# 0xPolygonZero/proof-protocol-decoder

Measured on NVIDIA B200. Metric: mpt_nodes_keccak_hashed_per_sec, higher is better.
Workload: dtype u64

## Files before the change

proof_protocol_decoder_b200/csrc/txn_core.h:

```cpp
#pragma once
#include <cstdint>

#include "../../include/ppd_flat.h"
#include "arena.h"

#if defined(__CUDACC__)
#define PPD_HD __host__ __device__ __forceinline__
#define PPD_INLINE
#else
#define PPD_HD
#define PPD_INLINE inline
#endif

namespace ppd {
namespace txn {

static const uint32_t T_UNCHANGED = 0xfffffffeu;
static const uint32_t ST_ABSENT = 0xfffffffeu;
static const uint32_t NONE = 0xfffffffdu;
static const uint32_t HASH_BASE = 0x80000000u, HASH_END = 0xf0000000u;
static const uint32_t MARK_SLOTS_T = 16;
static const uint32_t PATH_CAP = 15;
static const uint32_t OWNER_TXN_TRIE = 0xffffff01u, OWNER_RECEIPT_TRIE = 0xffffff02u, OWNER_STATE_TRIE = 0xffffff03u;
static const uint32_t TRF_STATE_WRITE = 0x100u;
// ... 202 lines not shown
#define PPD_PREFETCH(p) asm volatile("prefetch.global.L1 [%0];" ::"l"(p))
#define PPD_FENCE_BLOCK() __threadfence_block()
#define PPD_ATOMIC_SUB(p, x) atomicSub((p), (x))
#define PPD_ATOMIC_ADD(p, x) atomicAdd((p), (x))
#define PPD_ATOMIC_MAX(p, x) atomicMax((p), (x))
#define PPD_ATOMIC_CAS(p, c, x) atomicCAS((p), (c), (x))
#else
PPD_HD PPD_INLINE uint32_t host_atomic_add(uint32_t* p, uint32_t x) {
  uint32_t o = *p;
  *p = o + x;
  return o;
}
PPD_HD PPD_INLINE uint32_t host_atomic_max(uint32_t* p, uint32_t x) {
  uint32_t o = *p;
  if (x > o) *p = x;
  return o;
}
PPD_HD PPD_INLINE uint32_t host_atomic_cas(uint32_t* p, uint32_t c, uint32_t x) {
  uint32_t o = *p;
  if (o == c) *p = x;
  return o;
}
#define PPD_FENCE_BLOCK() ((void)0)
#define PPD_PREFETCH(p) ((void)0)
#define PPD_ATOMIC_SUB(p, x) ppd::txn::host_atomic_add((p), 0u - (x))
#define PPD_ATOMIC_ADD(p, x) ppd::txn::host_atomic_add((p), (x))
#define PPD_ATOMIC_MAX(p, x) ppd::txn::host_atomic_max((p), (x))
#define PPD_ATOMIC_CAS(p, c, x) ppd::txn::host_atomic_cas((p), (c), (x))
#endif

PPD_HD PPD_INLINE void raise(const View& v, uint32_t why, uint32_t txn) {
  if (PPD_ATOMIC_CAS(&v.cur->flag, 0u, why) == 0u) v.cur->flag_txn = txn;
}

PPD_HD PPD_INLINE uint32_t key_nib(const View& v, uint32_t koff, uint32_t i) {
  const uint32_t b = v.key_pool[koff + (i >> 1)];
  return (i & 1) ? (b & 15u) : (b >> 4);
}
PPD_HD PPD_INLINE uint32_t lvl(const View& v, uint32_t n) { return (n == NODE_EMPTY || n >= HASH_BASE) ? 0u : (uint32_t)v.level[n]; }
PPD_HD PPD_INLINE uint32_t kind_of(const View& v, uint32_t n) { return is_hash_id(n) ? (uint32_t)NK_HASH : (v.nodes[n].w0 & 0xffu); }
PPD_HD PPD_INLINE uint32_t w0(uint32_t kind, uint32_t start, uint32_t len) { return kind | (start << 8) | (len << 16); }

PPD_HD PPD_INLINE uint32_t push_node(const View& v, const NodeRec& r, uint32_t lv) {
  uint32_t id = PPD_ATOMIC_ADD(SCR(v).a_nodes, 1u);
  if (id >= v.cap_nodes) {
    raise(v, TXF_NODES_FULL, 0);
    id = v.cap_nodes - 1;
// ... 72 lines not shown
PPD_HD PPD_INLINE uint32_t child_at(const View& v, const NodeRec& br, uint32_t nib) {
  const uint32_t mask = br.a1 & 0xffffu, bit = 1u << nib;
  if (!(mask & bit)) return NODE_EMPTY;
#if defined(__CUDA_ARCH__)
  return v.child_pool[br.a0 + __popc(mask & (bit - 1))];
#else
  return v.child_pool[br.a0 + __builtin_popcount(mask & (bit - 1))];
#endif
}
PPD_HD PPD_INLINE uint32_t popc16(uint32_t m) {
#if defined(__CUDA_ARCH__)
  return __popc(m & 0xffffu);
#else
  return (uint32_t)__builtin_popcount(m & 0xffffu);
#endif
}

struct NL {
  uint32_t id, lv;
};
PPD_HD PPD_INLINE NL new_leaf_for(const View& v, const SOp& o, uint32_t start) {
  const uint32_t len = o.klen - start;
  if (o.kind == OP_PUT_ACCOUNT) {
    const uint32_t src = v.accounts[o.a1].storage_src;
    const uint32_t lv = src == NODE_EMPTY ? 0u : lvl(v, src) + 1u;
    return NL{push_node(v, NodeRec{w0(NK_LEAF_ACCOUNT, start, len), o.koff, o.a1, 0}, lv), lv};
  }
  return NL{push_node(v, NodeRec{w0(NK_LEAF, start, len), o.koff, o.a1, o.a2}, 0), 0};
}
PPD_HD PPD_INLINE NL new_ext(const View& v, uint32_t koff, uint32_t start, uint32_t len, NL child) {
  return NL{push_node(v, NodeRec{w0(NK_EXT, start, len), koff, child.id, 0}, child.lv + 1u), child.lv + 1u};
}
PPD_HD PPD_INLINE uint32_t new_root(const View& v, uint32_t child) {
  return push_node(v, NodeRec{w0(NK_ROOT, 0, 0), 0, child, 0}, child == NODE_EMPTY ? 0u : lvl(v, child) + 1u);
}
PPD_HD PPD_INLINE NL releaf(const View& v, uint32_t leaf, uint32_t leaf_lv, uint32_t koff, uint32_t start, uint32_t len) {
  NodeRec r = v.nodes[leaf];
  r.w0 = w0(r.w0 & 0xffu, start, len);
  r.a0 = koff;
  return NL{push_node(v, r, leaf_lv), leaf_lv};
}
PPD_HD PPD_INLINE NL new_branch16(const View& v, const uint32_t* kids, uint32_t lv) {
  uint32_t mask = 0, k = 0;
  for (uint32_t i = 0; i < 16; i++)
    if (kids[i] != NODE_EMPTY) mask |= 1u << i, k++;
  const uint32_t base = alloc_children(v, k);
  for (uint32_t i = 0, j = 0; i < 16; i++)
    if (kids[i] != NODE_EMPTY) v.child_pool[base + j++] = kids[i];
  return NL{push_node(v, NodeRec{w0(NK_BRANCH, 0, 0), base, mask, 0}, lv), lv};
}
PPD_HD PPD_INLINE NL branch_with(const View& v, uint32_t br, uint32_t nib, NL child) {
  const NodeRec r = v.nodes[br];
  uint32_t lv = v.level[br];
  const uint32_t mask = r.a1 & 0xffffu, bit = 1u << nib;
  const uint32_t k = popc16(mask), rk = popc16(mask & (bit - 1)), has = (mask & bit) ? 1u : 0u;
  const uint32_t nk = k - has + 1u, base = alloc_children(v, nk);
  uint32_t old[16];
  for (uint32_t i = 0; i < 16; i++) old[i] = i < k ? v.child_pool[r.a0 + i] : 0u;
  for (uint32_t i = 0; i < rk; i++) v.child_pool[base + i] = old[i];
  v.child_pool[base + rk] = child.id;
  for (uint32_t i = rk + has; i < k; i++) v.child_pool[base + i - has + 1u] = old[i];
  if (child.lv + 1u > lv) lv = child.lv + 1u;
  return NL{push_node(v, NodeRec{w0(NK_BRANCH, 0, 0), base, mask | bit, 0}, lv), lv};
}
PPD_HD PPD_INLINE NL collapse_ext(const View& v, uint32_t ek, uint32_t es, uint32_t el, NL child) {
  const uint32_t k = kind_of(v, child.id);
  if (k == NK_EXT) {
    const NodeRec c = v.nodes[child.id];
    return NL{push_node(v, NodeRec{w0(NK_EXT, ((c.w0 >> 8) & 0xffu) - el, ((c.w0 >> 16) & 0xffu) + el), c.a0, c.a1, 0}, child.lv), child.lv};
  }
  if (k == NK_LEAF || k == NK_LEAF_ACCOUNT) {
    const NodeRec c = v.nodes[child.id];
    return releaf(v, child.id, child.lv, c.a0, ((c.w0 >> 8) & 0xffu) - el, ((c.w0 >> 16) & 0xffu) + el);
  }
  return new_ext(v, ek, es, el, child);
}
PPD_HD PPD_INLINE NL collapse_branch(const View& v, uint32_t koff, uint32_t pos, uint32_t nib, NL other) {
  const uint32_t k = kind_of(v, other.id);
  if (k == NK_EXT || k == NK_LEAF || k == NK_LEAF_ACCOUNT) return collapse_ext(v, 0, pos, 1, other);
  const uint32_t nb = pos / 2 + 2;
  uint32_t pk = PPD_ATOMIC_ADD(SCR(v).a_keys, nb);
  if (pk + nb > v.cap_keys) {
    raise(v, TXF_KEYS_FULL, 0);
    pk = v.cap_keys - 40;
  }
  for (uint32_t i = 0; i <= pos / 2; i++) v.key_pool[pk + i] = v.key_pool[koff + i];
  uint8_t* last = v.key_pool + pk + pos / 2;
  *last = (pos & 1) ? (uint8_t)((*last & 0xf0u) | nib) : (uint8_t)(nib << 4);
  v.key_pool[pk + pos / 2 + 1] = 0;
  return new_ext(v, pk, pos, 1, other);
}

PPD_HD PPD_INLINE NL split_at(const View& v, const SOp& o, uint32_t pos, uint32_t cp, uint32_t existing_nib, NL existing, uint32_t txn) {
  const uint32_t at = pos + cp;
  if (at >= o.klen) {
    raise(v, TXF_KEY_PREFIX, txn);
    return existing;
  }
  const uint32_t new_nib = key_nib(v, o.koff, at);
  uint32_t kids[16];
  for (int i = 0; i < 16; i++) kids[i] = NODE_EMPTY;
  const NL leaf = new_leaf_for(v, o, at + 1);
  kids[existing_nib] = existing.id;
  kids[new_nib] = leaf.id;
  const NL br = new_branch16(v, kids, (existing.lv > leaf.lv ? existing.lv : leaf.lv) + 1u);
  return cp == 0 ? br : new_ext(v, o.koff, pos, cp, br);
}
PPD_HD PPD_INLINE NL insert_one(const View& v, NL base, uint32_t depth, const SOp& o, uint32_t txn) {
  uint32_t st_node[PATH_CAP + 1];
  uint8_t st_nib[PATH_CAP + 1];
  uint32_t sp = 0, node = base.id, pos = depth;
  NL result = base;
  for (;;) {
    if (node == NODE_EMPTY) {
      result = new_leaf_for(v, o, pos);
      break;
    }
    const uint32_t k = kind_of(v, node);
    if (k == NK_HASH || k == NK_ROOT) {
      raise(v, TXF_INSERT_INTO_HASH, txn);
      return base;
    }
    const NodeRec r = v.nodes[node];
    const uint32_t ns = (r.w0 >> 8) & 0xffu, nl = (r.w0 >> 16) & 0xffu;
    if (k == NK_BRANCH) {
      if (pos >= o.klen || sp == PATH_CAP + 1) {
        raise(v, pos >= o.klen ? TXF_KEY_PREFIX : TXF_STACK, txn);
        return base;
// ... 21 lines not shown
        break;
      }
    } else {
      const uint32_t avail = o.klen - pos, m = avail < nl ? avail : nl;
      const uint32_t cp = common_prefix(v, r.a0, ns, o.koff, pos, m);
      if (cp == nl && nl == avail) {
        result = new_leaf_for(v, o, pos);
      } else if (cp == nl) {
        raise(v, TXF_KEY_PREFIX, txn);
        return base;
      } else {
        const NL existing = releaf(v, node, node == base.id ? base.lv : (uint32_t)v.level[node], r.a0, ns + cp + 1, nl - cp - 1);
        result = split_at(v, o, pos, cp, key_nib(v, r.a0, ns + cp), existing, txn);
      }
      break;
    }
  }
  while (sp) {
    sp--;
    if (st_nib[sp] == 0xff) {
      const NodeRec r = v.nodes[st_node[sp]];
      result = new_ext(v, r.a0, (r.w0 >> 8) & 0xffu, (r.w0 >> 16) & 0xffu, result);
    } else {
      result = branch_with(v, st_node[sp], st_nib[sp], result);
    }
  }
  return result;
}

struct Batch {
  const SOp* ops;
  uint32_t n;
  uint32_t base;
  uint32_t txn;
};

PPD_HD PPD_INLINE int shared_depth(const Batch& b, uint32_t i) {
  const int prev = (int)b.ops[i].lcp, next = i + 1 < b.n ? (int)b.ops[i + 1].lcp : -1;
  return prev > next ? prev : next;
}
PPD_HD PPD_INLINE uint32_t trie_root_of(const View& v, uint32_t owner) {
  if (owner == OWNER_STATE_TRIE) return v.cur->state_root;
  if (owner == OWNER_TXN_TRIE) return v.cur->txn_root;
  if (owner == OWNER_RECEIPT_TRIE) return v.cur->receipt_root;
  return v.acct[v.traces[owner].acct].storage;
}

PPD_HD PPD_INLINE PathNode& pc_at(const View& v, uint32_t idx) { return idx < SCR(v).pc_n_fast ? SCR(v).pc_fast[idx] : SCR(v).pc_slow[idx - SCR(v).pc_n_fast]; }
PPD_HD PPD_INLINE uint32_t pc_hash(uint32_t node) { return node * 2654435761u; }
PPD_HD PPD_INLINE uint32_t pc_make(const View& v, uint32_t node, const NodeRec& r, bool is_branch, uint32_t owner, uint32_t txn) {
  uint32_t idx = PPD_ATOMIC_ADD(SCR(v).pc_count, 1u);
  if (idx >= SCR(v).pc_n_fast + SCR(v).pc_n_slow) {
    raise(v, TXF_PATH_TABLE, txn);
    return NONE;
  }
  PathNode& p = pc_at(v, idx);
  p.kids[0] = r.a0, p.kids[1] = is_branch ? (r.a1 & 0xffffu) : 0x10000u;
  p.node = node, p.lv = 0, p.pending = 0, p.owner = owner, p.changed = 0;
  uint32_t h = pc_hash(node) & SCR(v).pc_map_mask;
  for (;;) {
    const uint32_t prev = PPD_ATOMIC_CAS(&SCR(v).pc_map_key[h], 0xffffffffu, node);
    if (prev == 0xffffffffu || prev == node) break;
    h = (h + 1) & SCR(v).pc_map_mask;
  }
  SCR(v).pc_map[h] = idx + 1u;
  return idx;
}
PPD_HD PPD_INLINE void pc_fill(const View& v, uint32_t idx) {
  PathNode& p = pc_at(v, idx);
  const uint32_t a0 = p.kids[0], m = p.kids[1];
  const uint32_t old_lv = v.level[p.node];
  if (m & 0x10000u) {
    p.kids[0] = T_UNCHANGED, p.kids[1] = 0;
  } else {
    const uint32_t mask = m & 0xffffu;
    uint32_t x[16];
#if defined(__CUDA_ARCH__)
#pragma unroll
#endif
    for (uint32_t nib = 0; nib < 16; nib++) x[nib] = ((mask >> nib) & 1u) ? v.child_pool[a0 + popc16(mask & ((1u << nib) - 1u))] : NODE_EMPTY;
#if defined(__CUDA_ARCH__)
#pragma unroll
#endif
    for (uint32_t nib = 0; nib < 16; nib++) p.kids[nib] = x[nib];
  }
  p.lv = old_lv;
}
PPD_HD PPD_INLINE uint32_t pc_find(const View& v, uint32_t node) {
  uint32_t h = pc_hash(node) & SCR(v).pc_map_mask;
  for (;;) {
    const uint32_t k = SCR(v).pc_map_key[h];
    if (k == node) return SCR(v).pc_map[h] - 1u;
    if (k == 0xffffffffu) return NONE;
    h = (h + 1) & SCR(v).pc_map_mask;
  }
}

PPD_HD PPD_INLINE void batch_walk(const Ctx& c, const Batch& b, uint32_t i, uint32_t* touched) {
  const View& v = c.v;
  PPD_EV(v, b.txn, c.tid, 1);
  const SOp o = b.ops[i];
  const uint32_t e = b.base + i;
  uint32_t node = trie_root_of(v, o.owner), pos = 0, pl = 0, nt = 0;
  uint32_t kw[8];
  load_key_words(v, o.koff, (o.klen + 1u) >> 1, kw);
  uint32_t* pn = SCR(v).path_node + (size_t)e * PATH_CAP;
  uint8_t* pd = SCR(v).path_depth + (size_t)e * PATH_CAP;
  uint32_t tk = TK_EMPTY, tn = NODE_EMPTY, td = 0, tpc = NONE;
  const bool put = o.kind == OP_PUT_LEAF || o.kind == OP_PUT_ACCOUNT, mark = (o.pad & SOP_MARK) != 0;
  const int shared = shared_depth(b, i);
  for (;;) {
    if (node == NODE_EMPTY) {
      tk = TK_EMPTY, td = pos;
      break;
    }
    if (mark) touched[nt] = node;
    nt++;
    NodeRec r{NK_HASH, 0, 0, 0};
    if (!is_hash_id(node)) r = v.nodes[node];
    const uint32_t k = r.w0 & 0xffu;
    if (k == NK_HASH || k == NK_ROOT) {
      tk = TK_HASH, tn = node, td = pos;
      if (put) raise(v, TXF_INSERT_INTO_HASH, b.txn);
      if (mark && pos < o.klen) raise(v, TXF_MARK_INTO_HASH, b.txn);
      break;
    }
    const uint32_t ns = (r.w0 >> 8) & 0xffu, nl = (r.w0 >> 16) & 0xffu;
    const bool owner = (int)o.lcp < (int)pos && (int)pos <= shared;
    if (k == NK_BRANCH) {
      if (pos >= o.klen || pl == PATH_CAP) {
        if (pos >= o.klen) {
          if (put) raise(v, TXF_KEY_PREFIX, b.txn);
        } else {
          raise(v, TXF_PATH_DEPTH, b.txn);
        }
        tk = TK_BAD, tn = node, td = pos;
        break;
      }
      pn[pl] = node, pd[pl] = (uint8_t)pos, pl++;
      if (owner) pc_make(v, node, r, true, i, b.txn);
      node = child_at(v, r, nib_of_words(kw, pos));
      pos++;
    } else if (k == NK_EXT) {
      const uint32_t avail = o.klen - pos, m = avail < nl ? avail : nl;
      const uint32_t cp = common_prefix(v, r.a0, ns, o.koff, pos, m);
      if (owner) tpc = pc_make(v, node, r, false, i, b.txn);
      if (cp == nl) {
        if (pl == PATH_CAP) {
          raise(v, TXF_PATH_DEPTH, b.txn);
          tk = TK_BAD, tn = node, td = pos;
          break;
        }
        pn[pl] = node, pd[pl] = (uint8_t)(pos | 0x80u), pl++;
        node = r.a1;
        pos += nl;
      } else {
        if (cp == avail && put) raise(v, TXF_KEY_PREFIX, b.txn);
        tk = TK_DIVERGE, tn = node, td = pos;
        break;
      }
    } else {
      const uint32_t avail = o.klen - pos, m = avail < nl ? avail : nl;
      const uint32_t cp = common_prefix(v, r.a0, ns, o.koff, pos, m);
      const bool same = cp == nl && nl == avail;
      if (!same && (cp == nl || cp == avail) && put) raise(v, TXF_KEY_PREFIX, b.txn);
      tk = same ? TK_LEAF_SAME : TK_LEAF_OTHER, tn = node, td = pos;
      break;
    }
  }
  if (nt > MARK_SLOTS_T) raise(v, TXF_MARK_SLOTS, b.txn);
  SCR(v).plen[e] = (uint8_t)pl;
  SCR(v).tnode[e] = tn, SCR(v).tdepth[e] = (uint8_t)td, SCR(v).tkind[e] = (uint8_t)tk;
  SCR(v).key_hi[e] = (kw[0] << 24) | ((kw[0] & 0xff00u) << 8) | ((kw[0] >> 8) & 0xff00u) | (kw[0] >> 24);
  PPD_EV(v, b.txn, c.tid, 2);
}

static const uint32_t GROUP_MAX = 12;
PPD_HD PPD_INLINE bool build_group(const View& v, const Batch& b, uint32_t first, uint32_t end, uint32_t td, uint32_t old_leaf, bool keep_old, NL* out, uint32_t txn) {
  uint32_t ik[GROUP_MAX + 1], iop[GROUP_MAX + 1];
  int il[GROUP_MAX + 2];
  uint32_t m = 0;
  NodeRec oldr{};
  uint32_t old_koff = 0, old_lv = 0;
  if (keep_old) {
    oldr = v.nodes[old_leaf];
    old_koff = oldr.a0;
    old_lv = v.level[old_leaf];
    if (((oldr.w0 >> 8) & 0xffu) + ((oldr.w0 >> 16) & 0xffu) != 64u) return false;
  }
  bool old_placed = !keep_old;
  int run_min = 127, prev_cpx = -1;
  for (uint32_t j = first; j < end; j++) {
    if (j > first && (int)b.ops[j].lcp < run_min) run_min = b.ops[j].lcp;
    const uint8_t kind = b.ops[j].kind;
    if (kind != OP_PUT_LEAF && kind != OP_PUT_ACCOUNT) continue;
    if (b.ops[j].klen != 64 || m + 2 > GROUP_MAX) return false;
    int l_prev = m == 0 ? (int)td - 1 : run_min;
    if (!old_placed) {
      const int cpx = (int)td + (int)common_prefix(v, old_koff, td, b.ops[j].koff, td, 64 - td);
      if (cpx >= 64) return false;
      if (key_nib(v, old_koff, (uint32_t)cpx) < key_nib(v, b.ops[j].koff, (uint32_t)cpx)) {
        ik[m] = old_koff, iop[m] = NONE, il[m] = m == 0 ? (int)td - 1 : prev_cpx, m++;
        old_placed = true;
        l_prev = cpx;
      } else {
        prev_cpx = cpx;
      }
    }
    ik[m] = b.ops[j].koff, iop[m] = j, il[m] = l_prev, m++;
    run_min = 127;
  }
  if (!old_placed) ik[m] = old_koff, iop[m] = NONE, il[m] = m == 0 ? (int)td - 1 : prev_cpx, m++;
  il[m] = (int)td - 1;
  if (m == 0) {
    *out = NL{NODE_EMPTY, 0};
    return true;
  }
  uint32_t sd[GROUP_MAX + 1], slv[GROUP_MAX + 1], sk[GROUP_MAX + 1][16];
  uint32_t sp = 0;
  for (uint32_t k = 0; k < m; k++) {
    const int lc = il[k], ln = il[k + 1];
    const uint32_t s = (uint32_t)((lc > ln ? lc : ln) + 1);
    NL cur = iop[k] == NONE ? releaf(v, old_leaf, old_lv, old_koff, s, 64 - s) : new_leaf_for(v, b.ops[iop[k]], s);
    if (ln > lc) {
      sd[sp] = (uint32_t)ln, slv[sp] = cur.lv + 1u;
      for (int z = 0; z < 16; z++) sk[sp][z] = NODE_EMPTY;
      sk[sp][key_nib(v, ik[k], (uint32_t)ln)] = cur.id;
      sp++;
      continue;
    }
    if (sp == 0) {
      *out = cur;
      return true;
    }
    sk[sp - 1][key_nib(v, ik[k], (uint32_t)lc)] = cur.id;
    if (cur.lv + 1u > slv[sp - 1]) slv[sp - 1] = cur.lv + 1u;
    while (sp && (int)sd[sp - 1] > ln) {
      sp--;
      const uint32_t d = sd[sp];
      NL br = new_branch16(v, sk[sp], slv[sp]);
      const int parent = sp ? (int)sd[sp - 1] : (int)td - 1;
      const int p = parent > ln ? parent : ln;
      if (p < (int)d - 1) br = new_ext(v, ik[k], (uint32_t)(p + 1), d - (uint32_t)(p + 1), br);
      if (p < (int)td) {
        *out = br;
        return true;
      }
      const uint32_t nib = key_nib(v, ik[k], (uint32_t)p);
      if (sp && p == parent) {
        sk[sp - 1][nib] = br.id;
        if (br.lv + 1u > slv[sp - 1]) slv[sp - 1] = br.lv + 1u;
      } else {
        sd[sp] = (uint32_t)p, slv[sp] = br.lv + 1u;
        for (int z = 0; z < 16; z++) sk[sp][z] = NODE_EMPTY;
        sk[sp][nib] = br.id;
        sp++;
        break;
      }
    }
  }
  raise(v, TXF_STACK, txn);
  return false;
}

PPD_HD PPD_INLINE void batch_announce(const Ctx& c, const Batch& b, uint32_t i) {
  const View& v = c.v;
  const uint32_t e = b.base + i;
  const int lcp = (int)b.ops[i].lcp;
  const uint32_t pl = SCR(v).plen[e];
  const uint32_t* pn = SCR(v).path_node + (size_t)e * PATH_CAP;
  uint32_t* ppc = SCR(v).path_pc + (size_t)e * PATH_CAP;
  const uint8_t* pd = SCR(v).path_depth + (size_t)e * PATH_CAP;
  const int shared = shared_depth(b, i);
  bool leads = true;
  for (uint32_t t = pl; t-- > 0;) {
    const uint32_t d = pd[t] & 0x7fu;
    if ((int)d > shared) continue;
    const uint32_t child_depth = (pd[t] & 0x80u) ? (t + 1 < pl ? (uint32_t)(pd[t + 1] & 0x7fu) : (uint32_t)SCR(v).tdepth[e]) : d + 1;
    const uint32_t idx = pc_find(v, pn[t]);
    ppc[t] = idx;
    leads = leads && lcp < (int)child_depth;
    if (leads && idx != NONE) PPD_ATOMIC_ADD(&pc_at(v, idx).pending, 1u);
  }
  uint32_t tidx = NONE;
  if (SCR(v).tkind[e] == TK_DIVERGE && (int)SCR(v).tdepth[e] <= shared) {
    tidx = pc_find(v, SCR(v).tnode[e]);
    if (tidx != NONE) PPD_ATOMIC_ADD(&pc_at(v, tidx).pending, 1u);
  }
  SCR(v).tpc[e] = tidx;
}

PPD_HD PPD_INLINE NL assemble_branch(const View& v, PathNode& p, uint32_t koff, uint32_t d) {
  uint32_t nk = 0, last = 0;
  for (uint32_t nib = 0; nib < 16; nib++)
    if (p.kids[nib] != NODE_EMPTY) nk++, last = nib;
  if (nk >= 2) return new_branch16(v, p.kids, p.lv);
  if (nk == 1) return collapse_branch(v, koff, d, last, NL{p.kids[last], lvl(v, p.kids[last])});
  return NL{NODE_EMPTY, 0};
}
PPD_HD PPD_INLINE NL assemble_ext(const View& v, const Batch& b, PathNode& p, uint32_t d) {
  const NodeRec r = v.nodes[p.node];
  const uint32_t el = (r.w0 >> 16) & 0xffu;
  NL base{p.node, p.lv};
  bool changed = false;
  const uint32_t rj = p.kids[0];
  if (rj == NODE_EMPTY)
    base = NL{NODE_EMPTY, 0}, changed = true;
  else if (rj != T_UNCHANGED)
    base = collapse_ext(v, r.a0, d, el, NL{rj, p.kids[1]}), changed = true;
  for (uint32_t j = p.owner; j < b.n && (j == p.owner || (int)b.ops[j].lcp >= (int)d); j++)
    if (SCR(v).tkind[b.base + j] == TK_DIVERGE && SCR(v).tdepth[b.base + j] == d && (b.ops[j].kind == OP_PUT_LEAF || b.ops[j].kind == OP_PUT_ACCOUNT))
      base = insert_one(v, base, d, b.ops[j], b.txn), changed = true;
  return changed ? base : NL{T_UNCHANGED, 0};
}

PPD_HD PPD_INLINE void set_trie_root(const View& v, uint32_t owner, uint32_t r) {
  if (owner == OWNER_STATE_TRIE) {
    v.cur->state_root = r;
  } else if (owner == OWNER_TXN_TRIE) {
    v.cur->txn_root = r;
  } else if (owner == OWNER_RECEIPT_TRIE) {
    v.cur->receipt_root = r;
  } else {
    AcctState& a = v.acct[v.traces[owner].acct];
    a.storage = r, a.root_node = NONE;
  }
}

PPD_HD PPD_INLINE NL private_branch(const View& v, uint32_t node, uint32_t d, uint32_t nib, NL cur, uint32_t koff) {
  if (cur.id != NODE_EMPTY) return branch_with(v, node, nib, cur);
  const NodeRec r = v.nodes[node];
  const uint32_t lv = v.level[node];
  const uint32_t mask = r.a1 & 0xffffu, bit = 1u << nib;
  if (!(mask & bit)) return NL{T_UNCHANGED, 0};
  const uint32_t left = mask & ~bit, nk = popc16(left);
  if (nk >= 2) {
    const uint32_t base = alloc_children(v, nk), gone = popc16(mask & (bit - 1u));
    uint32_t old[16];
    for (uint32_t i = 0; i < 16; i++) old[i] = i <= nk ? v.child_pool[r.a0 + i] : 0u;
    for (uint32_t i = 0; i < nk; i++) v.child_pool[base + i] = old[i < gone ? i : i + 1u];
    return NL{push_node(v, NodeRec{w0(NK_BRANCH, 0, 0), base, left, 0}, lv), lv};
  }
  if (nk == 1) {
    const uint32_t last = ctz32(left), kid = v.child_pool[r.a0 + popc16(mask & ((1u << last) - 1u))];
    return collapse_branch(v, koff, d, last, NL{kid, lvl(v, kid)});
  }
  return NL{NODE_EMPTY, 0};
}
PPD_HD PPD_INLINE NL private_ext(const View& v, uint32_t node, uint32_t d, NL cur) {
  if (cur.id == NODE_EMPTY) return cur;
  const NodeRec r = v.nodes[node];
  return collapse_ext(v, r.a0, d, (r.w0 >> 16) & 0xffu, cur);
}

PPD_HD PPD_INLINE void batch_climb(const Ctx& c, const Batch& b, uint32_t i) {
  const View& v = c.v;
  const uint32_t e = b.base + i;
  const SOp& o = b.ops[i];
  const uint32_t tk = SCR(v).tkind[e], td = SCR(v).tdepth[e];
  const uint32_t* ppc = SCR(v).path_pc + (size_t)e * PATH_CAP;
  const uint8_t* pd = SCR(v).path_depth + (size_t)e * PATH_CAP;
  NL cur{T_UNCHANGED, 0};
  uint32_t t = SCR(v).plen[e];
  const int shared = shared_depth(b, i);
  if (tk == TK_DIVERGE && (int)td > shared) {
    if (o.kind == OP_PUT_LEAF || o.kind == OP_PUT_ACCOUNT) cur = insert_one(v, NL{SCR(v).tnode[e], (uint32_t)v.level[SCR(v).tnode[e]]}, td, o, b.txn);
  } else if (tk == TK_DIVERGE) {
    const uint32_t idx = SCR(v).tpc[e];
    if (idx == NONE) return;
    PathNode& p = pc_at(v, idx);
    PPD_FENCE_BLOCK();
    if (PPD_ATOMIC_SUB(&p.pending, 1u) != 1u) return;
    PPD_FENCE_BLOCK();
    cur = assemble_ext(v, b, p, td);
  } else {
    if ((int)o.lcp >= (int)td) return;
    if (tk == TK_EMPTY || tk == TK_LEAF_SAME || tk == TK_LEAF_OTHER) {
      bool any = false;
      for (uint32_t j = i; j < b.n && (j == i || (int)b.ops[j].lcp >= (int)td); j++) any |= b.ops[j].kind != OP_NONE;
      if (any) {
        NL base{NODE_EMPTY, 0};
        if (tk != TK_EMPTY) base = NL{SCR(v).tnode[e], (uint32_t)v.level[SCR(v).tnode[e]]};
        bool changed = false, keep_old = tk != TK_EMPTY;
        uint32_t end = i, n_put = 0;
        for (uint32_t j = i; j < b.n && (j == i || (int)b.ops[j].lcp >= (int)td); j++, end++) {
          const uint8_t kind = b.ops[j].kind;
          if (kind == OP_DEL && SCR(v).tkind[b.base + j] == TK_LEAF_SAME) base = NL{NODE_EMPTY, 0}, changed = true, keep_old = false;
          if (kind == OP_PUT_LEAF || kind == OP_PUT_ACCOUNT) {
            n_put++, changed = true;
            if (SCR(v).tkind[b.base + j] == TK_LEAF_SAME) keep_old = false;
          }
        }
        NL built;
        if (n_put >= 2 && build_group(v, b, i, end, td, SCR(v).tnode[e], keep_old, &built, b.txn)) {
          base = built;
        } else {
          for (uint32_t j = i; j < end; j++)
            if (b.ops[j].kind == OP_PUT_LEAF || b.ops[j].kind == OP_PUT_ACCOUNT) base = insert_one(v, base, td, b.ops[j], b.txn);
        }
        if (changed) cur = base;
      }
    }
  }
  PPD_EV(v, b.txn, c.tid, 11);
  for (;;) {
    if (t == 0) {
      if (cur.id != T_UNCHANGED) set_trie_root(v, o.owner, cur.id);
      return;
    }
    t--;
    const uint32_t d = pd[t] & 0x7fu;
    const bool is_ext = (pd[t] & 0x80u) != 0;
    if ((int)d > shared) {
      if (cur.id != T_UNCHANGED) {
        const uint32_t node = SCR(v).path_node[(size_t)e * PATH_CAP + t];
        cur = is_ext ? private_ext(v, node, d, cur) : private_branch(v, node, d, d < 8 ? (SCR(v).key_hi[e] >> (28 - 4 * d)) & 15u : key_nib(v, o.koff, d), cur, o.koff);
      }
      continue;
    }
    const uint32_t idx = ppc[t];
    if (idx == NONE) return;
    PathNode& q = pc_at(v, idx);
    if (cur.id != T_UNCHANGED) {
      if (is_ext) {
        q.kids[0] = cur.id, q.kids[1] = cur.lv;
      } else {
        q.kids[d < 8 ? (SCR(v).key_hi[e] >> (28 - 4 * d)) & 15u : key_nib(v, o.koff, d)] = cur.id;
        if (cur.id != NODE_EMPTY) PPD_ATOMIC_MAX(&q.lv, cur.lv + 1u);
      }
      q.changed = 1;
    }
    PPD_FENCE_BLOCK();
    if (PPD_ATOMIC_SUB(&q.pending, 1u) != 1u) return;
    PPD_FENCE_BLOCK();
    PPD_EV(v, b.txn, c.tid, 12);
    if (is_ext)
      cur = assemble_ext(v, b, q, d);
    else if (q.changed)
      cur = assemble_branch(v, q, o.koff, d);
    else
// ... 181 lines not shown
#define PPD_PHASE_CLOCK(c, k)                                \
  do {                                                       \
    if ((c).tid == 0) {                                      \
      const long long now_ = clock64();                      \
      (c).v.cur->phase_clocks[k] += now_ - *(c).sh_clock;    \
      *(c).sh_clock = now_;                                  \
    }                                                        \
  } while (0)
#else
#define PPD_BLOCK_SYNC() ((void)0)
#define PPD_PHASE_CLOCK(c, k) ((void)0)
#endif

PPD_HD PPD_INLINE void copy32(uint8_t* d, const uint8_t* s) {
  for (int i = 0; i < 32; i++) d[i] = s[i];
}

PPD_HD PPD_INLINE void run_txn(const Ctx& c, uint32_t ti, const uint8_t* empty_trie_hash, const uint8_t* empty_code_hash) {
  const View& v = c.v;
  const TxnDesc tx = v.txns[ti];
  const uint32_t ntr = tx.trace_end - tx.trace_begin;
  const uint32_t n1 = tx.op1_end - tx.op1_begin, n2 = tx.op2_end - tx.op2_begin;
  const SOp* ops1 = v.ops1 + tx.op1_begin;
  const SOp* ops2 = v.ops2 + tx.op2_begin;
  if (SCR(v).sh_ops) {
    for (uint32_t k = c.tid; k < n1 + n2; k += c.nthreads) SCR(v).sh_ops[k] = k < n1 ? ops1[k] : ops2[k - n1];
    ops1 = SCR(v).sh_ops, ops2 = SCR(v).sh_ops + n1;
  }
  if (c.tid == 0) {
    v.seg_b[tx.seg_tries + 0] = v.cur->state_root;
    v.seg_b[tx.seg_tries + 1] = v.cur->txn_root;
    v.seg_b[tx.seg_tries + 2] = v.cur->receipt_root;
    *SCR(v).pc_count = 0;
  }
  for (uint32_t k = c.tid; k <= SCR(v).pc_map_mask; k += c.nthreads) SCR(v).pc_map_key[k] = 0xffffffffu;
  for (uint32_t k = c.tid; k < ntr; k += c.nthreads) {
    const uint32_t t = tx.trace_begin + k;
    const TxnTrace& tr = v.traces[t];
    AcctState& a = v.acct[tr.acct];
    if (a.storage == ST_ABSENT) {
      uint32_t s = NODE_EMPTY;
      if (a.pre_rec != NONE && (v.pre_flags[a.pre_rec] & 1u) && tr.n_reads + tr.n_writes == 0) s = v.accounts[a.pre_rec].storage_src;
      a.storage = s, a.root_node = NONE;
    }
    v.seg_a[tx.seg_storage + 2 * tr.rank] = v.dig_base + 32u * t;
    v.seg_b[tx.seg_storage + 2 * tr.rank] = IR_SEG_KEY32;
    v.seg_a[tx.seg_storage + 2 * tr.rank + 1] = 0;
// ... 46 lines not shown
    const TxnTrace& tr = v.traces[t];
    if (!(tr.flags & TRF_STATE_WRITE)) continue;
    AccountRec rec;
    const uint32_t e = n1 + tr.rank;
    if (SCR(v).tkind[e] == TK_LEAF_SAME) {
      const uint32_t leaf = SCR(v).tnode[e];
      if ((v.nodes[leaf].w0 & 0xffu) != NK_LEAF_ACCOUNT) {
        raise(v, TXF_NOT_ACCOUNT, ti);
        continue;
      }
      rec = v.accounts[v.nodes[leaf].a1];
    } else {
      for (int i = 0; i < 32; i++) rec.nonce[i] = 0, rec.balance[i] = 0;
      copy32(rec.storage_root, empty_trie_hash);
      copy32(rec.code_hash, empty_code_hash);
      rec.storage_src = NODE_EMPTY;
      rec.pad[0] = rec.pad[1] = rec.pad[2] = 0;
    }
    if (tr.n_writes) {
      AcctState& a = v.acct[tr.acct];
      if (a.root_node == NONE) a.root_node = new_root(v, a.storage);
      rec.storage_src = a.root_node;
    }
    if (tr.flags & PPD_TR_BALANCE) copy32(rec.balance, v.flat + tr.off_balance);
    if (tr.flags & PPD_TR_NONCE) copy32(rec.nonce, v.flat + tr.off_nonce);
    if (tr.flags & PPD_TR_CODE_READ)
      copy32(rec.code_hash, v.flat + tr.code_off);
    else if (tr.flags & PPD_TR_CODE_WRITE)
      copy32(rec.code_hash, digest(v, tr.m_code));
    v.accounts[v.rec_base + tr.rec] = rec;
    PPD_EV(v, ti, c.tid, 31);
  }
  PPD_BLOCK_SYNC();
  PPD_PHASE_CLOCK(c, 4);
  if (c.tid == 0) PPD_EV(v, ti, 0, 100 + 4);
  for (uint32_t k = c.tid; k < n2; k += c.nthreads) {
    PPD_EV(v, ti, c.tid, 20);
    batch_climb(c, b2, k);
    PPD_EV(v, ti, c.tid, 24);
  }
  PPD_BLOCK_SYNC();
  PPD_PHASE_CLOCK(c, 5);
  if (c.tid == 0) PPD_EV(v, ti, 0, 100 + 5);
  for (uint32_t k = c.tid; k < ntr; k += c.nthreads) {
    const TxnTrace& tr = v.traces[tx.trace_begin + k];
    if (tr.flags & PPD_TR_SELF_DESTRUCTED) {
// ... 21 lines not shown
}
PPD_HD PPD_INLINE void run_finish(const Ctx& c, uint32_t initial_state) {
  const View& v = c.v;
  if (c.tid == 0 && !v.cur->flag) {
    Cursors& cur = *v.cur;
    cur.roots[XR_INITIAL_STATE] = new_root(v, initial_state);
    cur.roots[XR_EMPTY] = new_root(v, NODE_EMPTY);
    cur.roots[XR_FINAL_STATE] = new_root(v, cur.state_root);
    cur.roots[XR_FINAL_TXN] = new_root(v, cur.txn_root);
    cur.roots[XR_FINAL_RECEIPT] = new_root(v, cur.receipt_root);
    cur.state_before_withdrawals = cur.state_root;
    for (uint32_t w = 0; w < v.n_withdrawals && !cur.flag; w++) {
      const Withdrawal wd = v.withdrawals[w];
      const uint32_t koff = v.dig_base + 32u * wd.m_addr;
      const uint32_t leaf = get_leaf(v, cur.state_root, koff, 64);
      if (leaf == NODE_EMPTY || (v.nodes[leaf].w0 & 0xffu) != NK_LEAF_ACCOUNT) {
        raise(v, TXF_WITHDRAWAL, 0xffffffffu);
        break;
      }
      AccountRec rec = v.accounts[v.nodes[leaf].a1];
      u256_add(rec.balance, v.flat + wd.off_amount);
      v.accounts[v.rec_base + wd.rec] = rec;
      SOp o;
      o.koff = koff, o.klen = 64, o.lcp = -1, o.kind = OP_PUT_ACCOUNT, o.pad = 0, o.a1 = v.rec_base + wd.rec, o.a2 = 0, o.owner = OWNER_STATE_TRIE;
      cur.state_root = insert_one(v, NL{cur.state_root, lvl(v, cur.state_root)}, 0, o, 0xffffffffu).id;
    }
    cur.roots[XR_AFTER_WITHDRAWALS] = new_root(v, cur.state_root);
  }
  PPD_BLOCK_SYNC();
}

struct AcctExport {
  uint8_t haddr[32];
  uint32_t initial, final_;
};
PPD_HD PPD_INLINE void export_account(const View& v, const uint32_t* acct_list, const uint32_t* join_storage, uint32_t r, AcctExport* out) {
  const NodeRec nr = v.nodes[acct_list[5ull * r]];
  const uint32_t ns = (nr.w0 >> 8) & 0xffu, nl = (nr.w0 >> 16) & 0xffu, klen = ns + nl;
  AcctExport e;
  for (int i = 0; i < 32; i++) e.haddr[i] = 0;
  for (uint32_t k = 0; k < klen && k < 64; k++) {
    const uint32_t posn = 64 - klen + k, nib = key_nib(v, nr.a0, k);
    e.haddr[posn >> 1] |= (uint8_t)((posn & 1) ? nib : (nib << 4));
  }
  e.initial = join_storage[r];
  const uint32_t slot = v.pre_slot[r];
  e.final_ = slot < NONE ? v.acct[slot].storage : e.initial;
// ... 6 lines not shown
```

Before: 1.464 billion.

## Carry node levels and child rows through descent to cut dependent loads in climb

Node levels are now captured during descent and passed into pc_make, build_group and insert_one. Account-leaf levels are precomputed into the op's a2 field. For private path entries, the child-row base and the mask/level are stored in place of the node id, so climb no longer re-reads node records. Branch construction uses compact lists and a two-child helper instead of 16-slot arrays, and the child rows are prefetched before climbing. The aim is to remove dependent global loads and cut register and local-memory pressure, at the cost of more scratch writes and reusing a2 and tpc with more than one meaning.

```diff
diff --git a/proof_protocol_decoder_b200/csrc/txn_core.h b/proof_protocol_decoder_b200/csrc/txn_core.h
--- a/proof_protocol_decoder_b200/csrc/txn_core.h
+++ b/proof_protocol_decoder_b200/csrc/txn_core.h
@@ -248,7 +248,7 @@
   return o;
 }
 #define PPD_FENCE_BLOCK() ((void)0)
-#define PPD_PREFETCH(p) ((void)0)
+#define PPD_PREFETCH(p) ((void)(p))
 #define PPD_ATOMIC_SUB(p, x) ppd::txn::host_atomic_add((p), 0u - (x))
 #define PPD_ATOMIC_ADD(p, x) ppd::txn::host_atomic_add((p), (x))
 #define PPD_ATOMIC_MAX(p, x) ppd::txn::host_atomic_max((p), (x))
@@ -367,9 +367,7 @@
 PPD_HD PPD_INLINE NL new_leaf_for(const View& v, const SOp& o, uint32_t start) {
   const uint32_t len = o.klen - start;
   if (o.kind == OP_PUT_ACCOUNT) {
-    const uint32_t src = v.accounts[o.a1].storage_src;
-    const uint32_t lv = src == NODE_EMPTY ? 0u : lvl(v, src) + 1u;
-    return NL{push_node(v, NodeRec{w0(NK_LEAF_ACCOUNT, start, len), o.koff, o.a1, 0}, lv), lv};
+    return NL{push_node(v, NodeRec{w0(NK_LEAF_ACCOUNT, start, len), o.koff, o.a1, 0}, o.a2), o.a2};
   }
   return NL{push_node(v, NodeRec{w0(NK_LEAF, start, len), o.koff, o.a1, o.a2}, 0), 0};
 }
@@ -394,17 +392,34 @@
     if (kids[i] != NODE_EMPTY) v.child_pool[base + j++] = kids[i];
   return NL{push_node(v, NodeRec{w0(NK_BRANCH, 0, 0), base, mask, 0}, lv), lv};
 }
-PPD_HD PPD_INLINE NL branch_with(const View& v, uint32_t br, uint32_t nib, NL child) {
-  const NodeRec r = v.nodes[br];
-  uint32_t lv = v.level[br];
-  const uint32_t mask = r.a1 & 0xffffu, bit = 1u << nib;
+PPD_HD PPD_INLINE NL new_branch_list(const View& v, const uint8_t* nibs, const uint32_t* ids, uint32_t k, uint32_t lv) {
+  uint32_t mask = 0;
+  for (uint32_t i = 0; i < k; i++) mask |= 1u << nibs[i];
+  const uint32_t base = alloc_children(v, k);
+  for (uint32_t i = 0; i < k; i++) v.child_pool[base + i] = ids[i];
+  return NL{push_node(v, NodeRec{w0(NK_BRANCH, 0, 0), base, mask, 0}, lv), lv};
+}
+PPD_HD PPD_INLINE NL new_branch2(const View& v, uint32_t na, uint32_t a, uint32_t nb, uint32_t b, uint32_t lv) {
+  const uint32_t base = alloc_children(v, 2);
+  v.child_pool[base] = na < nb ? a : b;
+  v.child_pool[base + 1] = na < nb ? b : a;
+  return NL{push_node(v, NodeRec{w0(NK_BRANCH, 0, 0), base, (1u << na) | (1u << nb), 0}, lv), lv};
+}
+PPD_HD PPD_INLINE NL branch_with(const View& v, uint32_t a0, uint32_t mask, uint32_t lv, uint32_t nib, NL child) {
+  const uint32_t bit = 1u << nib;
   const uint32_t k = popc16(mask), rk = popc16(mask & (bit - 1)), has = (mask & bit) ? 1u : 0u;
   const uint32_t nk = k - has + 1u, base = alloc_children(v, nk);
-  uint32_t old[16];
-  for (uint32_t i = 0; i < 16; i++) old[i] = i < k ? v.child_pool[r.a0 + i] : 0u;
-  for (uint32_t i = 0; i < rk; i++) v.child_pool[base + i] = old[i];
+  uint32_t x[16];
+#if defined(__CUDA_ARCH__)
+#pragma unroll
+#endif
+  for (uint32_t i = 0; i < 16; i++) x[i] = i < k ? v.child_pool[a0 + i] : 0u;
+#if defined(__CUDA_ARCH__)
+#pragma unroll
+#endif
+  for (uint32_t i = 0; i < 16; i++)
+    if (i < k && (i < rk || i >= rk + has)) v.child_pool[base + (i < rk ? i : i - has + 1u)] = x[i];
   v.child_pool[base + rk] = child.id;
-  for (uint32_t i = rk + has; i < k; i++) v.child_pool[base + i - has + 1u] = old[i];
   if (child.lv + 1u > lv) lv = child.lv + 1u;
   return NL{push_node(v, NodeRec{w0(NK_BRANCH, 0, 0), base, mask | bit, 0}, lv), lv};
 }
@@ -443,12 +458,8 @@
     return existing;
   }
   const uint32_t new_nib = key_nib(v, o.koff, at);
-  uint32_t kids[16];
-  for (int i = 0; i < 16; i++) kids[i] = NODE_EMPTY;
   const NL leaf = new_leaf_for(v, o, at + 1);
-  kids[existing_nib] = existing.id;
-  kids[new_nib] = leaf.id;
-  const NL br = new_branch16(v, kids, (existing.lv > leaf.lv ? existing.lv : leaf.lv) + 1u);
+  const NL br = new_branch2(v, existing_nib, existing.id, new_nib, leaf.id, (existing.lv > leaf.lv ? existing.lv : leaf.lv) + 1u);
   return cp == 0 ? br : new_ext(v, o.koff, pos, cp, br);
 }
 PPD_HD PPD_INLINE NL insert_one(const View& v, NL base, uint32_t depth, const SOp& o, uint32_t txn) {
@@ -516,7 +527,8 @@
       const NodeRec r = v.nodes[st_node[sp]];
       result = new_ext(v, r.a0, (r.w0 >> 8) & 0xffu, (r.w0 >> 16) & 0xffu, result);
     } else {
-      result = branch_with(v, st_node[sp], st_nib[sp], result);
+      const NodeRec r = v.nodes[st_node[sp]];
+      result = branch_with(v, r.a0, r.a1 & 0xffffu, v.level[st_node[sp]], st_nib[sp], result);
     }
   }
   return result;
@@ -542,7 +554,7 @@
 
 PPD_HD PPD_INLINE PathNode& pc_at(const View& v, uint32_t idx) { return idx < SCR(v).pc_n_fast ? SCR(v).pc_fast[idx] : SCR(v).pc_slow[idx - SCR(v).pc_n_fast]; }
 PPD_HD PPD_INLINE uint32_t pc_hash(uint32_t node) { return node * 2654435761u; }
-PPD_HD PPD_INLINE uint32_t pc_make(const View& v, uint32_t node, const NodeRec& r, bool is_branch, uint32_t owner, uint32_t txn) {
+PPD_HD PPD_INLINE uint32_t pc_make(const View& v, uint32_t node, const NodeRec& r, uint32_t lv, bool is_branch, uint32_t owner, uint32_t txn) {
   uint32_t idx = PPD_ATOMIC_ADD(SCR(v).pc_count, 1u);
   if (idx >= SCR(v).pc_n_fast + SCR(v).pc_n_slow) {
     raise(v, TXF_PATH_TABLE, txn);
@@ -550,7 +562,7 @@
   }
   PathNode& p = pc_at(v, idx);
   p.kids[0] = r.a0, p.kids[1] = is_branch ? (r.a1 & 0xffffu) : 0x10000u;
-  p.node = node, p.lv = 0, p.pending = 0, p.owner = owner, p.changed = 0;
+  p.node = node, p.lv = lv, p.pending = 0, p.owner = owner, p.changed = 0;
   uint32_t h = pc_hash(node) & SCR(v).pc_map_mask;
   for (;;) {
     const uint32_t prev = PPD_ATOMIC_CAS(&SCR(v).pc_map_key[h], 0xffffffffu, node);
@@ -563,7 +575,6 @@
 PPD_HD PPD_INLINE void pc_fill(const View& v, uint32_t idx) {
   PathNode& p = pc_at(v, idx);
   const uint32_t a0 = p.kids[0], m = p.kids[1];
-  const uint32_t old_lv = v.level[p.node];
   if (m & 0x10000u) {
     p.kids[0] = T_UNCHANGED, p.kids[1] = 0;
   } else {
@@ -578,7 +589,6 @@
 #endif
     for (uint32_t nib = 0; nib < 16; nib++) p.kids[nib] = x[nib];
   }
-  p.lv = old_lv;
 }
 PPD_HD PPD_INLINE uint32_t pc_find(const View& v, uint32_t node) {
   uint32_t h = pc_hash(node) & SCR(v).pc_map_mask;
@@ -599,8 +609,9 @@
   uint32_t kw[8];
   load_key_words(v, o.koff, (o.klen + 1u) >> 1, kw);
   uint32_t* pn = SCR(v).path_node + (size_t)e * PATH_CAP;
+  uint32_t* pp = SCR(v).path_pc + (size_t)e * PATH_CAP;
   uint8_t* pd = SCR(v).path_depth + (size_t)e * PATH_CAP;
-  uint32_t tk = TK_EMPTY, tn = NODE_EMPTY, td = 0, tpc = NONE;
+  uint32_t tk = TK_EMPTY, tn = NODE_EMPTY, td = 0, tlv = 0;
   const bool put = o.kind == OP_PUT_LEAF || o.kind == OP_PUT_ACCOUNT, mark = (o.pad & SOP_MARK) != 0;
   const int shared = shared_depth(b, i);
   for (;;) {
@@ -611,7 +622,11 @@
     if (mark) touched[nt] = node;
     nt++;
     NodeRec r{NK_HASH, 0, 0, 0};
-    if (!is_hash_id(node)) r = v.nodes[node];
+    uint32_t lv = 0;
+    if (!is_hash_id(node)) {
+      r = v.nodes[node];
+      if ((int)pos > (int)o.lcp) lv = v.level[node];
+    }
     const uint32_t k = r.w0 & 0xffu;
     if (k == NK_HASH || k == NK_ROOT) {
       tk = TK_HASH, tn = node, td = pos;
@@ -621,6 +636,7 @@
     }
     const uint32_t ns = (r.w0 >> 8) & 0xffu, nl = (r.w0 >> 16) & 0xffu;
     const bool owner = (int)o.lcp < (int)pos && (int)pos <= shared;
+    const bool alone = (int)pos > shared;
     if (k == NK_BRANCH) {
       if (pos >= o.klen || pl == PATH_CAP) {
         if (pos >= o.klen) {
@@ -631,26 +647,34 @@
         tk = TK_BAD, tn = node, td = pos;
         break;
       }
-      pn[pl] = node, pd[pl] = (uint8_t)pos, pl++;
-      if (owner) pc_make(v, node, r, true, i, b.txn);
+      if (alone)
+        pn[pl] = r.a0, pp[pl] = (r.a1 & 0xffffu) | (lv << 16);
+      else
+        pn[pl] = node;
+      pd[pl] = (uint8_t)pos, pl++;
+      if (owner) pc_make(v, node, r, lv, true, i, b.txn);
       node = child_at(v, r, nib_of_words(kw, pos));
       pos++;
     } else if (k == NK_EXT) {
       const uint32_t avail = o.klen - pos, m = avail < nl ? avail : nl;
       const uint32_t cp = common_prefix(v, r.a0, ns, o.koff, pos, m);
-      if (owner) tpc = pc_make(v, node, r, false, i, b.txn);
+      if (owner) pc_make(v, node, r, lv, false, i, b.txn);
       if (cp == nl) {
         if (pl == PATH_CAP) {
           raise(v, TXF_PATH_DEPTH, b.txn);
           tk = TK_BAD, tn = node, td = pos;
           break;
         }
-        pn[pl] = node, pd[pl] = (uint8_t)(pos | 0x80u), pl++;
+        if (alone)
+          pn[pl] = r.a0, pp[pl] = nl | (lv << 16);
+        else
+          pn[pl] = node;
+        pd[pl] = (uint8_t)(pos | 0x80u), pl++;
         node = r.a1;
         pos += nl;
       } else {
         if (cp == avail && put) raise(v, TXF_KEY_PREFIX, b.txn);
-        tk = TK_DIVERGE, tn = node, td = pos;
+        tk = TK_DIVERGE, tn = node, td = pos, tlv = lv;
         break;
       }
     } else {
@@ -658,28 +682,29 @@
       const uint32_t cp = common_prefix(v, r.a0, ns, o.koff, pos, m);
       const bool same = cp == nl && nl == avail;
       if (!same && (cp == nl || cp == avail) && put) raise(v, TXF_KEY_PREFIX, b.txn);
-      tk = same ? TK_LEAF_SAME : TK_LEAF_OTHER, tn = node, td = pos;
+      tk = same ? TK_LEAF_SAME : TK_LEAF_OTHER, tn = node, td = pos, tlv = lv;
       break;
     }
   }
   if (nt > MARK_SLOTS_T) raise(v, TXF_MARK_SLOTS, b.txn);
   SCR(v).plen[e] = (uint8_t)pl;
   SCR(v).tnode[e] = tn, SCR(v).tdepth[e] = (uint8_t)td, SCR(v).tkind[e] = (uint8_t)tk;
+  SCR(v).tpc[e] = tlv;
   SCR(v).key_hi[e] = (kw[0] << 24) | ((kw[0] & 0xff00u) << 8) | ((kw[0] >> 8) & 0xff00u) | (kw[0] >> 24);
   PPD_EV(v, b.txn, c.tid, 2);
 }
 
 static const uint32_t GROUP_MAX = 12;
-PPD_HD PPD_INLINE bool build_group(const View& v, const Batch& b, uint32_t first, uint32_t end, uint32_t td, uint32_t old_leaf, bool keep_old, NL* out, uint32_t txn) {
+PPD_HD PPD_INLINE bool build_group(const View& v, const Batch& b, uint32_t first, uint32_t end, uint32_t td, uint32_t old_leaf, uint32_t old_lv, bool keep_old,
+                                   NL* out, uint32_t txn) {
   uint32_t ik[GROUP_MAX + 1], iop[GROUP_MAX + 1];
-  int il[GROUP_MAX + 2];
+  int8_t il[GROUP_MAX + 2];
   uint32_t m = 0;
   NodeRec oldr{};
-  uint32_t old_koff = 0, old_lv = 0;
+  uint32_t old_koff = 0;
   if (keep_old) {
     oldr = v.nodes[old_leaf];
     old_koff = oldr.a0;
-    old_lv = v.level[old_leaf];
     if (((oldr.w0 >> 8) & 0xffu) + ((oldr.w0 >> 16) & 0xffu) != 64u) return false;
   }
   bool old_placed = !keep_old;
@@ -694,45 +719,45 @@
       const int cpx = (int)td + (int)common_prefix(v, old_koff, td, b.ops[j].koff, td, 64 - td);
       if (cpx >= 64) return false;
       if (key_nib(v, old_koff, (uint32_t)cpx) < key_nib(v, b.ops[j].koff, (uint32_t)cpx)) {
-        ik[m] = old_koff, iop[m] = NONE, il[m] = m == 0 ? (int)td - 1 : prev_cpx, m++;
+        ik[m] = old_koff, iop[m] = NONE, il[m] = (int8_t)(m == 0 ? (int)td - 1 : prev_cpx), m++;
         old_placed = true;
         l_prev = cpx;
       } else {
         prev_cpx = cpx;
       }
     }
-    ik[m] = b.ops[j].koff, iop[m] = j, il[m] = l_prev, m++;
+    ik[m] = b.ops[j].koff, iop[m] = j, il[m] = (int8_t)l_prev, m++;
     run_min = 127;
   }
-  if (!old_placed) ik[m] = old_koff, iop[m] = NONE, il[m] = m == 0 ? (int)td - 1 : prev_cpx, m++;
-  il[m] = (int)td - 1;
+  if (!old_placed) ik[m] = old_koff, iop[m] = NONE, il[m] = (int8_t)(m == 0 ? (int)td - 1 : prev_cpx), m++;
+  il[m] = (int8_t)((int)td - 1);
   if (m == 0) {
     *out = NL{NODE_EMPTY, 0};
     return true;
   }
-  uint32_t sd[GROUP_MAX + 1], slv[GROUP_MAX + 1], sk[GROUP_MAX + 1][16];
-  uint32_t sp = 0;
+  uint32_t slv[GROUP_MAX + 1], eid[GROUP_MAX + 1];
+  uint8_t sd[GROUP_MAX + 1], sbeg[GROUP_MAX + 1], enib[GROUP_MAX + 1];
+  uint32_t sp = 0, ne = 0;
   for (uint32_t k = 0; k < m; k++) {
     const int lc = il[k], ln = il[k + 1];
     const uint32_t s = (uint32_t)((lc > ln ? lc : ln) + 1);
     NL cur = iop[k] == NONE ? releaf(v, old_leaf, old_lv, old_koff, s, 64 - s) : new_leaf_for(v, b.ops[iop[k]], s);
     if (ln > lc) {
-      sd[sp] = (uint32_t)ln, slv[sp] = cur.lv + 1u;
-      for (int z = 0; z < 16; z++) sk[sp][z] = NODE_EMPTY;
-      sk[sp][key_nib(v, ik[k], (uint32_t)ln)] = cur.id;
-      sp++;
+      sd[sp] = (uint8_t)ln, slv[sp] = cur.lv + 1u, sbeg[sp] = (uint8_t)ne, sp++;
+      enib[ne] = (uint8_t)key_nib(v, ik[k], (uint32_t)ln), eid[ne] = cur.id, ne++;
       continue;
     }
     if (sp == 0) {
       *out = cur;
       return true;
     }
-    sk[sp - 1][key_nib(v, ik[k], (uint32_t)lc)] = cur.id;
+    enib[ne] = (uint8_t)key_nib(v, ik[k], (uint32_t)lc), eid[ne] = cur.id, ne++;
     if (cur.lv + 1u > slv[sp - 1]) slv[sp - 1] = cur.lv + 1u;
     while (sp && (int)sd[sp - 1] > ln) {
       sp--;
       const uint32_t d = sd[sp];
-      NL br = new_branch16(v, sk[sp], slv[sp]);
+      NL br = new_branch_list(v, enib + sbeg[sp], eid + sbeg[sp], ne - sbeg[sp], slv[sp]);
+      ne = sbeg[sp];
       const int parent = sp ? (int)sd[sp - 1] : (int)td - 1;
       const int p = parent > ln ? parent : ln;
       if (p < (int)d - 1) br = new_ext(v, ik[k], (uint32_t)(p + 1), d - (uint32_t)(p + 1), br);
@@ -740,17 +765,13 @@
         *out = br;
         return true;
       }
-      const uint32_t nib = key_nib(v, ik[k], (uint32_t)p);
-      if (sp && p == parent) {
-        sk[sp - 1][nib] = br.id;
-        if (br.lv + 1u > slv[sp - 1]) slv[sp - 1] = br.lv + 1u;
-      } else {
-        sd[sp] = (uint32_t)p, slv[sp] = br.lv + 1u;
-        for (int z = 0; z < 16; z++) sk[sp][z] = NODE_EMPTY;
-        sk[sp][nib] = br.id;
-        sp++;
-        break;
-      }
+      const bool opens = !(sp && p == parent);
+      if (opens)
+        sd[sp] = (uint8_t)p, slv[sp] = br.lv + 1u, sbeg[sp] = (uint8_t)ne, sp++;
+      else if (br.lv + 1u > slv[sp - 1])
+        slv[sp - 1] = br.lv + 1u;
+      enib[ne] = (uint8_t)key_nib(v, ik[k], (uint32_t)p), eid[ne] = br.id, ne++;
+      if (opens) break;
     }
   }
   raise(v, TXF_STACK, txn);
@@ -776,12 +797,11 @@
     leads = leads && lcp < (int)child_depth;
     if (leads && idx != NONE) PPD_ATOMIC_ADD(&pc_at(v, idx).pending, 1u);
   }
-  uint32_t tidx = NONE;
   if (SCR(v).tkind[e] == TK_DIVERGE && (int)SCR(v).tdepth[e] <= shared) {
-    tidx = pc_find(v, SCR(v).tnode[e]);
+    const uint32_t tidx = pc_find(v, SCR(v).tnode[e]);
     if (tidx != NONE) PPD_ATOMIC_ADD(&pc_at(v, tidx).pending, 1u);
-  }
-  SCR(v).tpc[e] = tidx;
+    SCR(v).tpc[e] = tidx;
+  }
 }
 
 PPD_HD PPD_INLINE NL assemble_branch(const View& v, PathNode& p, uint32_t koff, uint32_t d) {
@@ -821,30 +841,46 @@
   }
 }
 
-PPD_HD PPD_INLINE NL private_branch(const View& v, uint32_t node, uint32_t d, uint32_t nib, NL cur, uint32_t koff) {
-  if (cur.id != NODE_EMPTY) return branch_with(v, node, nib, cur);
-  const NodeRec r = v.nodes[node];
-  const uint32_t lv = v.level[node];
-  const uint32_t mask = r.a1 & 0xffffu, bit = 1u << nib;
+PPD_HD PPD_INLINE NL private_branch(const View& v, uint32_t a0, uint32_t ml, uint32_t d, uint32_t nib, NL cur, uint32_t koff) {
+  const uint32_t mask = ml & 0xffffu, lv = ml >> 16;
+  if (cur.id != NODE_EMPTY) return branch_with(v, a0, mask, lv, nib, cur);
+  const uint32_t bit = 1u << nib;
   if (!(mask & bit)) return NL{T_UNCHANGED, 0};
   const uint32_t left = mask & ~bit, nk = popc16(left);
   if (nk >= 2) {
     const uint32_t base = alloc_children(v, nk), gone = popc16(mask & (bit - 1u));
-    uint32_t old[16];
-    for (uint32_t i = 0; i < 16; i++) old[i] = i <= nk ? v.child_pool[r.a0 + i] : 0u;
-    for (uint32_t i = 0; i < nk; i++) v.child_pool[base + i] = old[i < gone ? i : i + 1u];
+    uint32_t x[16];
+#if defined(__CUDA_ARCH__)
+#pragma unroll
+#endif
+    for (uint32_t i = 0; i < 16; i++) x[i] = i <= nk ? v.child_pool[a0 + i] : 0u;
+#if defined(__CUDA_ARCH__)
+#pragma unroll
+#endif
+    for (uint32_t i = 0; i < 16; i++)
+      if (i <= nk && i != gone) v.child_pool[base + (i < gone ? i : i - 1u)] = x[i];
     return NL{push_node(v, NodeRec{w0(NK_BRANCH, 0, 0), base, left, 0}, lv), lv};
   }
   if (nk == 1) {
-    const uint32_t last = ctz32(left), kid = v.child_pool[r.a0 + popc16(mask & ((1u << last) - 1u))];
+    const uint32_t last = ctz32(left), kid = v.child_pool[a0 + popc16(mask & ((1u << last) - 1u))];
     return collapse_branch(v, koff, d, last, NL{kid, lvl(v, kid)});
   }
   return NL{NODE_EMPTY, 0};
 }
-PPD_HD PPD_INLINE NL private_ext(const View& v, uint32_t node, uint32_t d, NL cur) {
+PPD_HD PPD_INLINE NL private_ext(const View& v, uint32_t ek, uint32_t ml, uint32_t d, NL cur) {
   if (cur.id == NODE_EMPTY) return cur;
-  const NodeRec r = v.nodes[node];
-  return collapse_ext(v, r.a0, d, (r.w0 >> 16) & 0xffu, cur);
+  return collapse_ext(v, ek, d, ml & 0xffffu, cur);
+}
+PPD_HD PPD_INLINE void prefetch_private_rows(const View& v, uint32_t e, uint32_t pl, int shared) {
+  const uint32_t* pn = SCR(v).path_node + (size_t)e * PATH_CAP;
+  const uint32_t* pp = SCR(v).path_pc + (size_t)e * PATH_CAP;
+  const uint8_t* pd = SCR(v).path_depth + (size_t)e * PATH_CAP;
+  for (uint32_t t = pl; t-- > 0 && (int)(pd[t] & 0x7fu) > shared;) {
+    if (pd[t] & 0x80u) continue;
+    const uint32_t* row = v.child_pool + pn[t];
+    PPD_PREFETCH(row);
+    PPD_PREFETCH(row + popc16(pp[t]) - 1u);
+  }
 }
 
 PPD_HD PPD_INLINE void batch_climb(const Ctx& c, const Batch& b, uint32_t i) {
@@ -852,13 +888,17 @@
   const uint32_t e = b.base + i;
   const SOp& o = b.ops[i];
   const uint32_t tk = SCR(v).tkind[e], td = SCR(v).tdepth[e];
+  const uint32_t* pn = SCR(v).path_node + (size_t)e * PATH_CAP;
   const uint32_t* ppc = SCR(v).path_pc + (size_t)e * PATH_CAP;
   const uint8_t* pd = SCR(v).path_depth + (size_t)e * PATH_CAP;
   NL cur{T_UNCHANGED, 0};
   uint32_t t = SCR(v).plen[e];
   const int shared = shared_depth(b, i);
   if (tk == TK_DIVERGE && (int)td > shared) {
-    if (o.kind == OP_PUT_LEAF || o.kind == OP_PUT_ACCOUNT) cur = insert_one(v, NL{SCR(v).tnode[e], (uint32_t)v.level[SCR(v).tnode[e]]}, td, o, b.txn);
+    if (o.kind == OP_PUT_LEAF || o.kind == OP_PUT_ACCOUNT) {
+      prefetch_private_rows(v, e, t, shared);
+      cur = insert_one(v, NL{SCR(v).tnode[e], SCR(v).tpc[e]}, td, o, b.txn);
+    }
   } else if (tk == TK_DIVERGE) {
     const uint32_t idx = SCR(v).tpc[e];
     if (idx == NONE) return;
@@ -873,8 +913,10 @@
       bool any = false;
       for (uint32_t j = i; j < b.n && (j == i || (int)b.ops[j].lcp >= (int)td); j++) any |= b.ops[j].kind != OP_NONE;
       if (any) {
+        prefetch_private_rows(v, e, t, shared);
+        const uint32_t tn = SCR(v).tnode[e], tlv = SCR(v).tpc[e];
         NL base{NODE_EMPTY, 0};
-        if (tk != TK_EMPTY) base = NL{SCR(v).tnode[e], (uint32_t)v.level[SCR(v).tnode[e]]};
+        if (tk != TK_EMPTY) base = NL{tn, tlv};
         bool changed = false, keep_old = tk != TK_EMPTY;
         uint32_t end = i, n_put = 0;
         for (uint32_t j = i; j < b.n && (j == i || (int)b.ops[j].lcp >= (int)td); j++, end++) {
@@ -886,7 +928,7 @@
           }
         }
         NL built;
-        if (n_put >= 2 && build_group(v, b, i, end, td, SCR(v).tnode[e], keep_old, &built, b.txn)) {
+        if (n_put >= 2 && build_group(v, b, i, end, td, tn, tlv, keep_old, &built, b.txn)) {
           base = built;
         } else {
           for (uint32_t j = i; j < end; j++)
@@ -906,10 +948,9 @@
     const uint32_t d = pd[t] & 0x7fu;
     const bool is_ext = (pd[t] & 0x80u) != 0;
     if ((int)d > shared) {
-      if (cur.id != T_UNCHANGED) {
-        const uint32_t node = SCR(v).path_node[(size_t)e * PATH_CAP + t];
-        cur = is_ext ? private_ext(v, node, d, cur) : private_branch(v, node, d, d < 8 ? (SCR(v).key_hi[e] >> (28 - 4 * d)) & 15u : key_nib(v, o.koff, d), cur, o.koff);
-      }
+      if (cur.id != T_UNCHANGED)
+        cur = is_ext ? private_ext(v, pn[t], ppc[t], d, cur)
+                     : private_branch(v, pn[t], ppc[t], d, d < 8 ? (SCR(v).key_hi[e] >> (28 - 4 * d)) & 15u : key_nib(v, o.koff, d), cur, o.koff);
       continue;
     }
     const uint32_t idx = ppc[t];
@@ -1137,7 +1178,7 @@
   const uint32_t ntr = tx.trace_end - tx.trace_begin;
   const uint32_t n1 = tx.op1_end - tx.op1_begin, n2 = tx.op2_end - tx.op2_begin;
   const SOp* ops1 = v.ops1 + tx.op1_begin;
-  const SOp* ops2 = v.ops2 + tx.op2_begin;
+  SOp* ops2 = v.ops2 + tx.op2_begin;
   if (SCR(v).sh_ops) {
     for (uint32_t k = c.tid; k < n1 + n2; k += c.nthreads) SCR(v).sh_ops[k] = k < n1 ? ops1[k] : ops2[k - n1];
     ops1 = SCR(v).sh_ops, ops2 = SCR(v).sh_ops + n1;
@@ -1230,6 +1271,7 @@
       if (a.root_node == NONE) a.root_node = new_root(v, a.storage);
       rec.storage_src = a.root_node;
     }
+    ops2[tr.rank].a2 = rec.storage_src == NODE_EMPTY ? 0u : lvl(v, rec.storage_src) + 1u;
     if (tr.flags & PPD_TR_BALANCE) copy32(rec.balance, v.flat + tr.off_balance);
     if (tr.flags & PPD_TR_NONCE) copy32(rec.nonce, v.flat + tr.off_nonce);
     if (tr.flags & PPD_TR_CODE_READ)
@@ -1297,7 +1339,8 @@
       u256_add(rec.balance, v.flat + wd.off_amount);
       v.accounts[v.rec_base + wd.rec] = rec;
       SOp o;
-      o.koff = koff, o.klen = 64, o.lcp = -1, o.kind = OP_PUT_ACCOUNT, o.pad = 0, o.a1 = v.rec_base + wd.rec, o.a2 = 0, o.owner = OWNER_STATE_TRIE;
+      o.koff = koff, o.klen = 64, o.lcp = -1, o.kind = OP_PUT_ACCOUNT, o.pad = 0, o.a1 = v.rec_base + wd.rec, o.owner = OWNER_STATE_TRIE;
+      o.a2 = rec.storage_src == NODE_EMPTY ? 0u : lvl(v, rec.storage_src) + 1u;
       cur.state_root = insert_one(v, NL{cur.state_root, lvl(v, cur.state_root)}, 0, o, 0xffffffffu).id;
     }
     cur.roots[XR_AFTER_WITHDRAWALS] = new_root(v, cur.state_root);
```

Result: no change. 1.454 billion, median of 6 (-0.7%).
